# mgp25/OpenLTE

Measured on AMD Instinct MI355X. Metric: DL subframes/sec @20MHz 100RB 64QAM, full chain FFT->CE->demap->rate-unmatch->turbo(REF)->CRC (SURVEY 8d W4), higher is better.
Workload: dtype i8 IQ in, f32 FFT/CE/equaliser, i8 soft bits, i16 path metrics (differences exact modulo 2^16); 1 GPU; W4 full DL chain: 20 MHz/100 RB/64QAM, 9 allocations per subframe (8x12 PRB TBS 3240 + 1x4 PRB TBS 1064), 65536 subframes per GPU, int8 IQ in HBM; subframes_per_gpu=65536, N_ant=1, CFI=2, channel_estimate_form=compact, decoder=REF (reference-faithful, bit-exact), unique_subframes=96, streams_per_gpu=1

## Files before the change

openlte_amd/csrc/turbo.hip:

```cpp
#include <algorithm>
#include <cstring>
#include <type_traits>
#include <vector>

#include "plan_core.hpp"

namespace {

constexpr uint32_t RX_NULL_AS_INT = 10000;

__host__ __device__ inline uint32_t kpad64(uint32_t K) { return (K + 63u) & ~63u; }


__device__ __forceinline__ int sbyte(uint32_t w, int k) { return (int)__builtin_amdgcn_sbfe(w, 8 * k, 8); }

typedef __attribute__((address_space(3))) const uint8_t  lds_u8_t;
typedef __attribute__((address_space(3))) const int8_t   lds_i8_t;
typedef __attribute__((address_space(3))) const uint16_t lds_u16_t;
__device__ __forceinline__ uint32_t lds_u8(uint32_t addr) { return *(lds_u8_t *)(uintptr_t)addr; }
__device__ __forceinline__ int      lds_i8(uint32_t addr) { return *(lds_i8_t *)(uintptr_t)addr; }
__device__ __forceinline__ uint32_t lds_u16(uint32_t addr) { return *(lds_u16_t *)(uintptr_t)addr; }

typedef short v2s __attribute__((ext_vector_type(2)));
__device__ __forceinline__ v2s      as_v2s(uint32_t w) { return __builtin_bit_cast(v2s, w); }
__device__ __forceinline__ uint32_t as_u32(v2s v) { return __builtin_bit_cast(uint32_t, v); }
__device__ __forceinline__ v2s      even2(uint32_t w) { return (as_v2s(w) << 8) >> 8; }
__device__ __forceinline__ v2s      odd2(uint32_t w) { return as_v2s(w) >> 8; }
__device__ __forceinline__ uint32_t merge_bytes(v2s e, v2s o) { return __builtin_amdgcn_perm(as_u32(o), as_u32(e), 0x06020400u); }
__device__ __forceinline__ v2s      abs2(v2s a) { return __builtin_elementwise_max(a, (v2s)(0) - a); }
__device__ __forceinline__ uint32_t neg_mask(v2s d)
{
    uint32_t m;
    asm("v_pk_ashrrev_i16 %0, 15, %1 op_sel_hi:[0,1]" : "=v"(m) : "v"(as_u32(d)));
    return m;
}
__device__ __forceinline__ v2s bit_select(uint32_t m, v2s yes, v2s no) { return as_v2s((as_u32(yes) & m) | (as_u32(no) & ~m)); }
__device__ __forceinline__ v2s half_sum(v2s a, v2s b)
{
    uint32_t t = as_u32(a + b);
    asm("" : "+v"(t));
    return as_v2s(t) >> 1;
}

__device__ __forceinline__ int soft_xor(int a, int b)
{
    int mag = (abs(a) + abs(b)) >> 1;
    return ((a < 0) != (b < 0)) ? -mag : mag;
}


template <typename Op> __device__ __forceinline__ int wave_reduce_i(int v, Op op)
{
    v = op(v, __builtin_amdgcn_update_dpp(v, v, 0xB1, 0xF, 0xF, false));
    v = op(v, __builtin_amdgcn_update_dpp(v, v, 0x4E, 0xF, 0xF, false));
    v = op(v, __builtin_amdgcn_update_dpp(v, v, 0x141, 0xF, 0xF, false));
    v = op(v, __builtin_amdgcn_update_dpp(v, v, 0x140, 0xF, 0xF, false));
// ... 188 lines not shown
            nulls = __popc(mask0) + __popc(mask0 & lowmask(c + 1)) + __popc(mask2 & lowmask(cc));
        }
        cn = p - nulls;
    }
};

struct CbDesc { uint32_t alloc, e_off, E, combo, Nnn, hard, tbs, pad; };

struct GroupDesc {
    const mi_lte_pdsch_alloc *allocs;
    const uint32_t *cb_alloc;
    const int8_t   *e_base;
    const uint32_t *e_off;
    const uint32_t *e_len;
    uint8_t        *out_bits;
    uint32_t        out_stride;
    int32_t        *status;
    const uint32_t *crc_tab;
    uint32_t        ul;
    uint32_t        packed;
    const CbDesc   *desc;
};

struct KSeg {
    uint32_t        K, n_cb, cb_base, n_tiles;
    uint32_t        wg_cb;
    uint32_t        wg_perm, perm_grid;
    uint32_t        e_cap;
    uint32_t        wv1, wv23;
    uint64_t        arr_off;
    __attribute__((address_space(1))) const uint16_t *pi, *inv2, *tabs;
    __attribute__((address_space(1))) const uint32_t *nnn;
    uint32_t        ws1, ws23;
    uint64_t        pad;
};
static_assert(sizeof(KSeg) == 96, "KSeg is read with scalar loads: keep it a multiple of 16 bytes");
struct MultiArgs { const KSeg *segs; const uint32_t *map; };
typedef __attribute__((address_space(4))) const KSeg     const_seg_t;
typedef __attribute__((address_space(4))) const uint32_t const_map_t;
__device__ __forceinline__ const_seg_t &multi_seg(const MultiArgs &ma, uint32_t slot)
{
    const uint32_t idx = reinterpret_cast<const_map_t *>(reinterpret_cast<uintptr_t>(ma.map))[__builtin_amdgcn_readfirstlane(slot)];
    return reinterpret_cast<const_seg_t *>(reinterpret_cast<uintptr_t>(ma.segs))[idx];
}


struct SrcRateUnmatch {
    static constexpr bool kIntegerValued = true;
    uint32_t e_cap;
    GroupDesc       g;
    const uint16_t *tabs;
    const uint32_t *nnn;
    const uint16_t *tab;
    const int8_t   *e;
    uint32_t        E, Nnn, K_;
    __device__ __forceinline__ void seg(const_seg_fwd_t &sg);
    __device__ __forceinline__ void init(uint32_t cb, uint32_t K)
    {
        const_u32x4_t *dp = reinterpret_cast<const_u32x4_t *>(reinterpret_cast<uintptr_t>(g.desc + cb));
        const u32x4_t  d0 = dp[0], d1 = dp[1];
        tab = tabs + (size_t)d0.w * 3 * K;
        Nnn = d1.x;
        K_  = K;
        e   = g.e_base + (size_t)d0.y * 64;
        E   = d0.z;
        hard = d1.y != 0;
    }
// ... 912 lines not shown
        }
        __syncthreads();
        uint4 I1 = make_uint4(0, 0, 0, 0);
        if (nv > 0) {
            uint32_t idx[16];
            unpack_idx16(praw, idx);
            I1 = gather16_bytes(MTAB_N, idx);
        }
        if (nv >= 0) *reinterpret_cast<uint4 *>(a.out[0] + unit_off(tile_off, lane, u)) = I1;
        uint32_t w[16], wm = 0;
        if (nv <= 0) X2 = make_uint4(0, 0, 0, 0);
        abs_sum16(X2, I1, w, wm);
        const int   wmax = block_max_i((int)wm, red_i);
        if (wmax == 254 || wmax == 127) {
            uint32_t o[4];
#pragma unroll
            for (int j = 0; j < 4; j++) {
                const uint32_t p = pack4u(w[4 * j], w[4 * j + 1], w[4 * j + 2], w[4 * j + 3]);
                o[j] = wmax == 254 ? (p >> 1) & 0x7F7F7F7Fu : p;
            }
            if (nv >= 0) *reinterpret_cast<uint4 *>(a.out[1] + unit_off(tile_off, lane, u)) = make_uint4(o[0], o[1], o[2], o[3]);
            continue;
        }
        const float W = (float)wmax;
        for (uint32_t t = threadIdx.x; t < MTAB_N; t += blockDim.x) mtab[t] = (int8_t)(int)(127.0f * ((float)t / W));
        __syncthreads();
        if (nv >= 0) *reinterpret_cast<uint4 *>(a.out[1] + unit_off(tile_off, lane, u)) = lookup16(0, w);
        __syncthreads();
    }
}

struct VoteArgs { const uint8_t *X0, *A1, *B1, *B2; };

template <bool GROUP, int NSLOT, bool MULTI = false>
__global__ __launch_bounds__(384) __attribute__((amdgpu_waves_per_eu(6, 8))) void k_turbo_vote(VoteArgs a, uint32_t K_arg, uint32_t n_cb_arg, const uint16_t *__restrict__ inv_arg,
                                                    uint8_t *__restrict__ c_bits, GroupDesc g, MultiArgs ma)
{
    static_assert(NSLOT == 1, "one unit per thread");
    uint32_t K = K_arg, n_cb = n_cb_arg, bidx = blockIdx.x;
    size_t   seg_off = 0;
    const uint16_t *__restrict__ inv = inv_arg;
    if constexpr (MULTI) {
        const_seg_t &sg = multi_seg(ma, blockIdx.x >> 9);
        K = sg.K; n_cb = sg.n_cb; inv = (const uint16_t *)sg.inv2; bidx = blockIdx.x - sg.wg_cb; seg_off = sg.arr_off;
        g.desc += sg.cb_base;
    }
    extern __shared__ __attribute__((aligned(16))) int8_t sm[];
    const uint32_t cb = xcd_cb(bidx, n_cb), tile = cb >> 6, lane = cb & 63, Kp = kpad64(K), n_units = Kp >> 4;
    if (cb >= n_cb) return;
    const size_t   tile_off = seg_off + (size_t)tile * Kp * 64;
    int8_t        *d12 = sm, *bits = sm + 2 * Kp + 32;
    uint32_t      *red_u = reinterpret_cast<uint32_t *>(bits + Kp);
    const uint32_t u  = threadIdx.x;
    const int      nv = (u < n_units) ? min(16, max(0, (int)K - 16 * (int)u)) : -1;
    IdxRaw vraw;
    {
        const uint4 *ip = reinterpret_cast<const uint4 *>(inv + 16 * (size_t)(nv > 0 ? u : 0));
        vraw.lo = ip[0];
        vraw.hi = ip[1];
    }
    const uint32_t crc_w0 = (GROUP && nv > 0) ? g.crc_tab[MI_CRC_TAB_BIAS + K - 16 * u - 16] : 0u;
    v2s            s0e[4], s0o[4];
    if (threadIdx.x == 0) *reinterpret_cast<uint32_t *>(d12 + 2 * Kp) = 0u;
    if (nv >= 0) {
        const UnitWords wa = load_unit_words(a.A1, tile_off, lane, u), wb = load_unit_words(a.B1, tile_off, lane, u),
                        wc = load_unit_words(a.B2, tile_off, lane, u);
        WordPairs       pa = word_pairs(wa.w[0]), pb = word_pairs(wb.w[0]), pc = word_pairs(wc.w[0]);
        const uint4    x0 = *reinterpret_cast<const uint4 *>(a.X0 + unit_off(tile_off, lane, u));
        const uint32_t x0w[4] = {x0.x, x0.y, x0.z, x0.w};
        uint32_t       dn[8];
#pragma unroll
        for (int j = 0; j < 4; j++) {
            const WordPairs ca = word_pairs(wa.w[j + 1]), cb1 = word_pairs(wb.w[j + 1]), cb2 = word_pairs(wc.w[j + 1]);
            SX              fe, fo, ge, go, he, ho;
            feedback_sm(ca, pa, fe, fo);
            feedback_sm(cb1, pb, ge, go);
            feedback_sm(cb2, pc, he, ho);
            v2s d[2];
#pragma unroll
            for (int h = 0; h < 2; h++) {
                const SM  &A = h ? ca.o : ca.e, &B = h ? cb1.o : cb1.e, &B_ = h ? cb2.o : cb2.e;
                const SX  &G = h ? go : ge, &G_ = h ? ho : he;
                const v2s  At = h ? ca.ot : ca.et;
                const v2s dAG = At - G.tc, t = as_v2s(as_u32(dAG) ^ B.s) - as_v2s(B.s);
                const v2s v1  = bit_select(B.s ^ G.s, (v2s)(0) - (t >> 1), half_sum(B.m, G.m));
                const v2s v2  = bit_select(B_.s ^ G_.s, (v2s)(0) - ((B_.m - G_.tc) >> 1), half_sum(B_.m, G_.m));
                d[h] = v1 + v2;
                const v2s c1 = sxor_tc(A, h ? fo : fe);
                (h ? s0o[j] : s0e[j]) = (h ? odd2(x0w[j]) : even2(x0w[j])) + c1;
            }
            pa = ca; pb = cb1; pc = cb2;
            const bool in = 4 * j < nv;
            dn[2 * j]     = in ? __builtin_amdgcn_perm(as_u32(d[1]), as_u32(d[0]), 0x05040100u) : 0u;
            dn[2 * j + 1] = in ? __builtin_amdgcn_perm(as_u32(d[1]), as_u32(d[0]), 0x07060302u) : 0u;
        }
        uint4 *dst = reinterpret_cast<uint4 *>(d12 + 32 * u);
        dst[0] = make_uint4(dn[0], dn[1], dn[2], dn[3]);
        dst[1] = make_uint4(dn[4], dn[5], dn[6], dn[7]);
    } else {
#pragma unroll
        for (int j = 0; j < 4; j++) s0e[j] = s0o[j] = (v2s)(0);
    }
    __syncthreads();
    uint32_t alloc = 0, tbs = 0, F = 0, crc = 0;
    if (GROUP) {
        alloc = g.desc[cb].alloc;
        tbs   = g.desc[cb].tbs;
        F     = K - tbs - 24;
    }
    if (nv > 0) {
        const uint32_t  iw[8] = {vraw.lo.x, vraw.lo.y, vraw.lo.z, vraw.lo.w, vraw.hi.x, vraw.hi.y, vraw.hi.z, vraw.hi.w};
        uint32_t        me[4], mo[4], bw[4];
#pragma unroll
        for (int j = 0; j < 4; j++) {
            const uint32_t i0 = iw[2 * j] & 0xFFFFu, i1 = iw[2 * j] >> 16, i2 = iw[2 * j + 1] & 0xFFFFu, i3 = iw[2 * j + 1] >> 16;
            const uint32_t ge = lds_u16(i0) | lds_u16(i2) << 16, go = lds_u16(i1) | lds_u16(i3) << 16;
            me[j] = as_u32((s0e[j] + as_v2s(ge)) >> 15);
            mo[j] = as_u32((s0o[j] + as_v2s(go)) >> 15);
            bw[j] = (me[j] & 0x00010001u) | (mo[j] & 0x00010001u) << 8;
        }
        if (GROUP) {
            if (!(nv == 16 && 16 * u >= F)) {
#pragma unroll
                for (int j = 0; j < 4; j++) {
                    auto ok = [&](int k) { return (k < nv && 16 * u + k >= F) ? 0xFFFFu : 0u; };
                    me[j] &= ok(4 * j) | ok(4 * j + 2) << 16;
                    mo[j] &= ok(4 * j + 1) | ok(4 * j + 3) << 16;
                }
            }
            const uint32_t GS = 0x864CFBu << 8;
            uint32_t       w = crc_w0;
#pragma unroll
            for (int k = 15; k >= 0; k--) {
                const int      j = k >> 2;
                const uint32_t m = (k & 3) == 0 ? (uint32_t)__builtin_amdgcn_sbfe(me[j], 0, 1) : (k & 3) == 1 ? (uint32_t)__builtin_amdgcn_sbfe(mo[j], 0, 1)
                                 : (k & 3) == 2 ? (uint32_t)((int)me[j] >> 31) : (uint32_t)((int)mo[j] >> 31);
                crc ^= w & m;
                if (k > 0) w = (w << 1) ^ ((uint32_t)((int)w >> 31) & GS);
            }
        }
        const uint4 pk = make_uint4(bw[0], bw[1], bw[2], bw[3]);
        if (GROUP) *reinterpret_cast<uint4 *>(bits + 16 * u) = pk;
        else {
            uint2 *o = reinterpret_cast<uint2 *>(c_bits + (size_t)cb * K + 16 * u);
            o[0] = make_uint2(pk.x, pk.y);
            if (nv > 8) o[1] = make_uint2(pk.z, pk.w);
        }
    }
    if (GROUP) {
        crc = wave_xor_u(crc);
        __syncthreads();
        if ((threadIdx.x & 63) == 0) red_u[threadIdx.x >> 6] = crc;
        __syncthreads();
        crc = 0;
        for (uint32_t w = 0; w < (blockDim.x >> 6); w++) crc ^= red_u[w];
        if (threadIdx.x == 0) g.status[alloc] = (crc == 0) ? 0  : 2 ;
        uint8_t *o = g.out_bits + (size_t)alloc * g.out_stride;
        if (g.packed && ((F | tbs) & 7u) == 0) {
            const uint32_t nby = tbs >> 3, nw = nby >> 2;
            auto byte_at = [&](uint32_t m) -> uint32_t {
                const uint2 w = *reinterpret_cast<const uint2 *>(bits + F + 8 * m);
                return (((w.x * 0x08040201u) >> 24) & 0xFu) << 4 | (((w.y * 0x08040201u) >> 24) & 0xFu);
            };
            for (uint32_t m = threadIdx.x; m < nw; m += blockDim.x)
                reinterpret_cast<uint32_t *>(o)[m] = byte_at(4 * m) | byte_at(4 * m + 1) << 8 | byte_at(4 * m + 2) << 16 | byte_at(4 * m + 3) << 24;
            for (uint32_t m = 4 * nw + threadIdx.x; m < nby; m += blockDim.x) o[m] = (uint8_t)byte_at(m);
        } else if (g.packed) {
            for (uint32_t m = threadIdx.x; m < (tbs + 7) >> 3; m += blockDim.x) {
                uint32_t v = 0;
                for (uint32_t b = 0; b < 8; b++) v = v << 1 | ((8 * m + b < tbs) ? ((uint32_t)bits[F + 8 * m + b] & 1u) : 0u);
                o[m] = (uint8_t)v;
            }
        } else if ((F & 3u) == 0) {
            const uint32_t nq = tbs >> 2;
            const uint32_t *bw = reinterpret_cast<const uint32_t *>(bits + F);
            for (uint32_t m = threadIdx.x; m < nq; m += blockDim.x) reinterpret_cast<uint32_t *>(o)[m] = bw[m];
            for (uint32_t m = 4 * nq + threadIdx.x; m < tbs; m += blockDim.x) o[m] = (uint8_t)bits[m + F];
        } else
            for (uint32_t m = threadIdx.x; m < tbs; m += blockDim.x) o[m] = (uint8_t)bits[m + F];
    }
}

__global__ __launch_bounds__(256) void k_cb_desc(GroupDesc g, uint32_t n_cb, const uint32_t *__restrict__ nnn, CbDesc *__restrict__ out)
{
    const uint32_t cb = blockIdx.x * blockDim.x + threadIdx.x;
    if (cb >= n_cb) return;
    const uint32_t a = g.cb_alloc[cb], txm = g.allocs[a].tx_mode;
    const uint32_t combo = g.ul ? 8u + (g.allocs[a].rv_idx & 3u)
                                : ((g.allocs[a].rv_idx & 3u) << 1) | ((txm == 3 || txm == 4 || txm == 8 || txm == 9) ? 1u : 0u);
    CbDesc d;
    d.alloc = a; d.e_off = g.e_off[a]; d.E = g.e_len[a]; d.combo = combo; d.Nnn = nnn[combo];
    d.hard  = (g.allocs[a].mod_type >= 2 && d.E <= d.Nnn) ? 1u : 0u;
    d.tbs   = g.allocs[a].tbs; d.pad = 0;
    out[cb] = d;
}

__global__ __launch_bounds__(256) void k_cb_desc_multi(GroupDesc g, uint32_t n_cb, const KSeg *__restrict__ segs, uint32_t n_seg, CbDesc *__restrict__ out)
{
    const uint32_t cb = blockIdx.x * blockDim.x + threadIdx.x;
    if (cb >= n_cb) return;
    uint32_t lo = 0, hi = n_seg;
    while (hi - lo > 1) {
        const uint32_t mid = (lo + hi) >> 1;
        if (segs[mid].cb_base <= cb) lo = mid; else hi = mid;
    }
    const uint32_t a = g.cb_alloc[cb], txm = g.allocs[a].tx_mode;
    const uint32_t combo = g.ul ? 8u + (g.allocs[a].rv_idx & 3u)
                                : ((g.allocs[a].rv_idx & 3u) << 1) | ((txm == 3 || txm == 4 || txm == 8 || txm == 9) ? 1u : 0u);
    CbDesc d;
    d.alloc = a; d.e_off = g.e_off[a]; d.E = g.e_len[a]; d.combo = combo; d.Nnn = segs[lo].nnn[combo];
    d.hard  = (g.allocs[a].mod_type >= 2 && d.E <= d.Nnn) ? 1u : 0u;
    d.tbs   = g.allocs[a].tbs; d.pad = 0;
// ... 229 lines not shown

static bool no_static_lds(const void *kernel)
{
    hipFuncAttributes a;
    return hipFuncGetAttributes(&a, kernel) == hipSuccess && a.sharedSizeBytes == 0;
}

struct RefScratch {
    uint8_t *base;
    CbDesc  *d_desc;
    PrepOut  po;
    SisoArgs s1, s23;
    PermArgs pa;
    VoteArgs va;
    RefScratch(void *scratch, size_t arr_bytes) : base((uint8_t *)scratch)
    {
        uint8_t *arr[N_BYTE_ARRAYS];
        for (int a = 0; a < N_BYTE_ARRAYS; a++) arr[a] = base + a * arr_bytes;
        uint32_t *dec[3];
        for (int p = 0; p < 3; p++) dec[p] = (uint32_t *)(base + N_BYTE_ARRAYS * arr_bytes + p * (arr_bytes / 2));
        d_desc = (CbDesc *)(base + N_BYTE_ARRAYS * arr_bytes + 3 * (arr_bytes / 2));
        po.arr[0] = arr[AX0]; po.arr[1] = arr[AX1]; po.arr[2] = arr[AX2];
        po.arr[3] = arr[AI0]; po.arr[4] = arr[AM1]; po.arr[5] = arr[AM2];
        s1.p[0] = {arr[AX1], arr[AX0], arr[AM1], arr[AA1], dec[0]};
        s1.p[1] = s1.p[0];
        pa.A1 = arr[AA1]; pa.X2 = arr[AX2]; pa.out[0] = arr[AI1]; pa.out[1] = arr[AM3];
        s23.p[0] = {arr[AX2], arr[AI0], arr[AM2], arr[AB1], dec[1]};
        s23.p[1] = {arr[AX2], arr[AI1], arr[AM3], arr[AB2], dec[2]};
        va = {arr[AX0], arr[AA1], arr[AB1], arr[AB2]};
    }
};
static uint32_t gpw_of(uint32_t n_tr) { return n_tr <= 2048 ? 1u : n_tr <= 4096 ? 2u : n_tr <= 8192 ? 4u : SMALL_G; }

template <typename Src, bool GROUP>
static int turbo_ref_run(mi_lte_ctx *ctx, Src src, uint32_t K, uint32_t n_cb, uint8_t *d_c_bits, GroupDesc gd, uint32_t e_cap = 0)
{
    TurboTables tb;
    int         rc = mi_ctx_turbo_tables(ctx, K, 0, &tb);
    if (rc != MI_LTE_OK) return rc;
    static const bool lds_ok = no_static_lds((const void *)k_turbo_prep<Src, 1>) && no_static_lds((const void *)k_turbo_perm<1>) &&
                               no_static_lds((const void *)k_turbo_vote<GROUP, 1>);
    if (!lds_ok) {
        ctx->err = "turbo kernels were built with static LDS: absolute LDS addressing is invalid";
        return MI_LTE_ERR_HIP;
    }
    const size_t n_tiles = (n_cb + 63) / 64, Kp = kpad64(K), arr_bytes = n_tiles * Kp * 64;
    rc = mi_ctx_reserve_scratch(ctx, mi_lte_turbo_scratch_bytes(K, n_cb));
    if (rc != MI_LTE_OK) return rc;
    const RefScratch sc(ctx->scratch, arr_bytes);
    const bool small = n_cb <= ctx->siso_small_max;
    if (n_cb % 64 && !small)
        MI_HIP_CHECK(ctx, hipMemsetAsync(sc.base, 0, N_BYTE_ARRAYS * arr_bytes, ctx->stream));

    if constexpr (GROUP) {
        gd.desc = src.g.desc = sc.d_desc;
        MI_LAUNCH(ctx, "k_cb_desc", k_cb_desc, dim3((n_cb + 255) / 256), dim3(256), 0, gd, n_cb, (const uint32_t *)src.nnn, sc.d_desc);
    }
    const uint32_t cb_threads = (uint32_t)(((Kp >> 4) + 63) & ~(size_t)63);
    MI_LAUNCH(ctx, "k_turbo_prep", (k_turbo_prep<Src, 1>), dim3(8 * xcd_chunk(n_cb)), dim3(cb_threads), prep_lds_bytes(Kp, e_cap), src, K, n_cb, tb.d_pi, sc.po, MultiArgs{});

    auto lds_of = [&](uint32_t gpw) { return sizeof(uint32_t) * gpw * (64 * 4 * 2 + (Kp >> 5) * 4); };
    if (small)
        MI_LAUNCH(ctx, "k_turbo_siso_small", k_turbo_siso_small<false>, dim3((n_cb + gpw_of(n_cb) - 1) / gpw_of(n_cb)), dim3(64), lds_of(gpw_of(n_cb)), sc.s1, K, n_cb, 0u,
                  gpw_of(n_cb), MultiArgs{});
    else
        MI_LAUNCH(ctx, "k_turbo_siso", k_turbo_siso<false>, dim3(((n_tiles + 1) / 2 + 3) / 4), dim3(256), 0, sc.s1, K, (uint32_t)n_tiles, 0u, MultiArgs{}, (const uint32_t *)nullptr);

    const uint32_t perm_grid = ((8 * xcd_chunk(n_cb) + PERM_NB - 1) / PERM_NB + 7u) & ~7u;
    MI_LAUNCH(ctx, "k_turbo_perm", k_turbo_perm<1>, dim3(perm_grid), dim3(cb_threads), MTAB_N + Kp + 32, sc.pa, K, n_cb, tb.d_pi, MultiArgs{});

    if (small)
        MI_LAUNCH(ctx, "k_turbo_siso_small", k_turbo_siso_small<false>, dim3((2 * n_cb + gpw_of(2 * n_cb) - 1) / gpw_of(2 * n_cb)), dim3(64), lds_of(gpw_of(2 * n_cb)), sc.s23, K,
                  n_cb, 1u, gpw_of(2 * n_cb), MultiArgs{});
    else
        MI_LAUNCH(ctx, "k_turbo_siso", k_turbo_siso<false>, dim3((n_tiles + 3) / 4), dim3(256), 0, sc.s23, K, (uint32_t)n_tiles, 1u, MultiArgs{}, (const uint32_t *)nullptr);

    MI_LAUNCH(ctx, "k_turbo_vote", (k_turbo_vote<GROUP, 1>), dim3(8 * xcd_chunk(n_cb)), dim3(cb_threads), 3 * Kp + 64, sc.va, K, n_cb, tb.d_inv2, d_c_bits, gd, MultiArgs{});
    MI_HIP_CHECK(ctx, hipGetLastError());
    ctx->last_kernels = "k_turbo_prep:1,k_turbo_siso:2,k_turbo_perm:1,k_turbo_vote:1";
    return MI_LTE_OK;
}

template <typename T>
static int turbo_ref_batch(mi_lte_ctx *ctx, const T *d_soft, uint32_t K, uint32_t n_cb, uint8_t *d_c_bits)
{
    SrcDirect<T> src{0, d_soft, nullptr};
    GroupDesc    none{};
    return turbo_ref_run<SrcDirect<T>, false>(ctx, src, K, n_cb, d_c_bits, none);
}

static int rm_rank_tables(mi_lte_ctx *ctx, uint32_t K, RmTables *out)
{
    auto it = ctx->rm_tables.find(K);
    if (it == ctx->rm_tables.end()) {
        RmTables t;
        MI_HIP_CHECK(ctx, hipMalloc((void **)&t.d_tabs, sizeof(uint16_t) * 12 * 3 * K));
        MI_HIP_CHECK(ctx, hipMalloc((void **)&t.d_nnn, sizeof(uint32_t) * 12));
        ctx->owned.push_back(t.d_tabs);
        ctx->owned.push_back(t.d_nnn);
        MI_LAUNCH(ctx, "k_rm_rank_table", k_rm_rank_table, dim3((3 * K + 255) / 256, 12), dim3(256), 0, K, t.d_tabs, t.d_nnn);
        MI_HIP_CHECK(ctx, hipGetLastError());
        it = ctx->rm_tables.emplace(K, t).first;
    }
    *out = it->second;
    return MI_LTE_OK;
}

static GroupDesc group_desc(const mi_lte_ctx *ctx, const MiDecodeIO &io, uint32_t cb_base = 0)
{
    return {io.d_allocs, io.d_cb_alloc + cb_base, io.d_e, io.d_e_off, io.d_e_len, io.d_out_bits, io.out_stride, io.d_status, ctx->d_crc_tab, io.ul ? 1u : 0u, io.packed ? 1u : 0u};
}
static uint32_t stage_cap(uint32_t e_max_bytes) { return (e_max_bytes + 16u + 63u) & ~63u; }

static bool mi_turbo_ref_multi_takes(uint32_t K, uint32_t e_max_bytes) { return (e_max_bytes + (3 * K - 81) - 1) / (3 * K - 81) <= 258; }

static int mi_turbo_ref_group(mi_lte_ctx *ctx, const MiKGroup &gr, const MiDecodeIO &io)
{
    int rc = mi_ctx_crc_table(ctx);
    if (rc != MI_LTE_OK) return rc;
    const GroupDesc gd = group_desc(ctx, io, gr.cb_base);
    RmTables rt;
    rc = rm_rank_tables(ctx, gr.K, &rt);
    if (rc != MI_LTE_OK) return rc;
    SrcRateUnmatch src;
    src.g    = gd;
    src.tabs = rt.d_tabs;
    src.nnn  = rt.d_nnn;
    const uint32_t cap = stage_cap(gr.e_max);
    src.e_cap          = (prep_lds_bytes(kpad64(gr.K), cap) <= 48 * 1024) ? cap : 0;
    if (mi_turbo_ref_multi_takes(gr.K, gr.e_max)) {
        SrcRateUnmatchPk pk;
        static_cast<SrcRateUnmatch &>(pk) = src;
        return turbo_ref_run<SrcRateUnmatchPk, true>(ctx, pk, gr.K, gr.n_cb, nullptr, gd, src.e_cap);
    }
    return turbo_ref_run<SrcRateUnmatch, true>(ctx, src, gr.K, gr.n_cb, nullptr, gd, src.e_cap);
}

static int mi_turbo_ref_multi(mi_lte_ctx *ctx, const MiKGroup *groups, uint32_t n_groups, const MiDecodeIO &io, MiMultiCache *cache)
{
    if (!groups || n_groups == 0 || n_groups > 0xFFFF || !cache) return MI_LTE_ERR_INVALID_ARG;
    int rc = mi_ctx_crc_table(ctx);
    if (rc != MI_LTE_OK) return rc;
    static const bool lds_ok = no_static_lds((const void *)k_turbo_prep<SrcRateUnmatchPk, 1, true>) && no_static_lds((const void *)k_turbo_perm<1, true>) &&
                               no_static_lds((const void *)k_turbo_vote<true, 1, true>);
    if (!lds_ok) { ctx->err = "turbo kernels were built with static LDS: absolute LDS addressing is invalid"; return MI_LTE_ERR_HIP; }
    constexpr int NCLS = 6;
    auto cls_of = [](uint32_t K) { return (int)((((kpad64(K) >> 4) + 63) >> 6) - 1); };
    const bool same = cache->built_for.size() == n_groups && memcmp(cache->built_for.data(), groups, sizeof(MiKGroup) * n_groups) == 0;
    if (!same) {
        cache->built_for.clear();
        std::vector<KSeg>     segs(n_groups);
        std::vector<uint32_t> map;
        MiMultiGeom          &G = cache->geom;
        G = MiMultiGeom{};
        uint64_t arr = 0;
        uint32_t cbs = 0;
        for (uint32_t i = 0; i < n_groups; i++) {
            const MiKGroup &gr = groups[i];
            if ((i && gr.K <= groups[i - 1].K) || gr.n_cb == 0) { ctx->err = "merged decode: groups must be non-empty and in ascending block size"; return MI_LTE_ERR_INVALID_ARG; }
            TurboTables tb;
            RmTables    rt;
            if ((rc = mi_ctx_turbo_tables(ctx, gr.K, 0, &tb)) != MI_LTE_OK || (rc = rm_rank_tables(ctx, gr.K, &rt)) != MI_LTE_OK) return rc;
            KSeg &sg = segs[i];
            memset(&sg, 0, sizeof(sg));
            const uint32_t Kp = kpad64(gr.K), cap = stage_cap(gr.e_max);
            sg.K = gr.K; sg.n_cb = gr.n_cb; sg.cb_base = gr.cb_base; sg.n_tiles = (gr.n_cb + 63) / 64;
            const uint32_t cap_w = (uint32_t)((15 * (size_t)(gr.K + 4) / 4 + 64 + 63) & ~(size_t)63);
            sg.e_cap = (prep_lds_bytes(Kp, cap) <= 48 * 1024) ? (Kp <= 1024 ? std::min(cap, cap_w) : cap) : cap_w;
            sg.arr_off = arr;
            typedef __attribute__((address_space(1))) const uint16_t gl16_t;
            typedef __attribute__((address_space(1))) const uint32_t gl32_t;
            sg.pi = (gl16_t *)tb.d_pi; sg.inv2 = (gl16_t *)tb.d_inv2; sg.tabs = (gl16_t *)rt.d_tabs; sg.nnn = (gl32_t *)rt.d_nnn;
            arr += (uint64_t)sg.n_tiles * Kp * 64;
            cbs = std::max(cbs, gr.cb_base + gr.n_cb);
            const int c = cls_of(gr.K);
            G.one_size[c] = (G.lds_prep[c] == 0 && gr.n_cb % 64 == 0) ? (int)i : -1;
            G.off_one[c] = sg.arr_off; G.e_cap_one[c] = sg.e_cap;
// ... 48 lines not shown
            const uint32_t n_wg = (n_wv + 3) / 4;
            if (!many_sizes || n_wg < 512) return;
            *at = (uint32_t)map.size();
            for (uint32_t j = 0; j < n_wg; j++) {
                const uint32_t round = j / 256, c = j % 256, in_round = std::min(256u, n_wg - 256 * round);
                const uint32_t src = (round & 1u) ? 256 * round + (in_round - 1 - std::min(c, in_round - 1)) : j;
                for (uint32_t t = 0; t < 4; t++) map.push_back(4 * src + t < n_wv ? 4 * src + t : 0xFFFFFFFFu);
            }
            *n_out = 4 * n_wg;
        };
        deal(G.n_wv1, &G.ord_wv1, &G.n_ord1);
        deal(G.n_wv23, &G.ord_wv23, &G.n_ord23);
        uint32_t tot = 0, kp_all = 0;
        for (uint32_t i = 0; i < n_groups; i++) { tot += groups[i].n_cb; kp_all = std::max(kp_all, kpad64(groups[i].K)); }
        G.gpw1 = gpw_of(tot); G.gpw23 = gpw_of(2 * tot); G.kp_all = kp_all;
        G.map_ws1 = (uint32_t)map.size();
        uint32_t wg = 0;
        for (uint32_t i = 0; i < n_groups; i++) {
            const uint32_t n = (groups[i].n_cb + G.gpw1 - 1) / G.gpw1;
            segs[i].ws1 = wg;
            map.insert(map.end(), n, i);
            wg += n;
        }
        G.n_ws1   = wg;
        G.map_ws23 = (uint32_t)map.size();
        wg = 0;
        for (uint32_t i = 0; i < n_groups; i++) {
            const uint32_t n = (2 * groups[i].n_cb + G.gpw23 - 1) / G.gpw23;
            segs[i].ws23 = wg;
            map.insert(map.end(), n, i);
            wg += n;
        }
        G.n_ws23 = wg;
        const size_t seg_bytes = sizeof(KSeg) * n_groups, map_bytes = (sizeof(uint32_t) * map.size() + 15) & ~(size_t)15, need = seg_bytes + map_bytes;
        if (need > cache->cap) {
            MI_HIP_CHECK(ctx, hipStreamSynchronize(ctx->stream));
            if (cache->d_tab) (void)hipFree(cache->d_tab);
            cache->d_tab = nullptr; cache->cap = 0;
            MI_HIP_CHECK(ctx, hipMalloc(&cache->d_tab, need + need / 4));
            cache->cap = need + need / 4;
        }
        std::vector<uint8_t> blob(need, 0);
        memcpy(blob.data(), segs.data(), seg_bytes);
        memcpy(blob.data() + seg_bytes, map.data(), sizeof(uint32_t) * map.size());
        MI_H2D(ctx, cache->d_tab, blob.data(), need);
        G.map_off = seg_bytes;
        cache->built_for.assign(groups, groups + n_groups);
    }
    const MiMultiGeom &G = cache->geom;
    const size_t A = G.arr_bytes;
    rc = mi_ctx_reserve_scratch(ctx, N_BYTE_ARRAYS * A + 3 * (A / 2) + (size_t)((G.n_slots + 63) & ~63u) * sizeof(CbDesc));
    if (rc != MI_LTE_OK) return rc;
    const RefScratch sc(ctx->scratch, A);
    const KSeg     *d_segs = (const KSeg *)cache->d_tab;
    const uint32_t *d_map  = (const uint32_t *)((const uint8_t *)cache->d_tab + G.map_off);

    GroupDesc gd = group_desc(ctx, io);
    gd.desc = sc.d_desc;
    MI_LAUNCH(ctx, "k_cb_desc", k_cb_desc_multi, dim3((G.n_slots + 255) / 256), dim3(256), 0, gd, G.n_slots, d_segs, n_groups, sc.d_desc);
    SrcRateUnmatchPk src;
    src.g = gd; src.tabs = nullptr; src.nnn = nullptr; src.e_cap = 0;
    for (int c = 0; c < NCLS; c++)
        if (G.grid_cb[c]) {
            if (G.one_size[c] >= 0) {
                const MiKGroup &gr = groups[G.one_size[c]];
                TurboTables tb;
                RmTables    rt;
                if ((rc = mi_ctx_turbo_tables(ctx, gr.K, 0, &tb)) != MI_LTE_OK || (rc = rm_rank_tables(ctx, gr.K, &rt)) != MI_LTE_OK) return rc;
                SrcRateUnmatchPk s1 = src;
                s1.tabs = rt.d_tabs; s1.nnn = rt.d_nnn; s1.g.desc = sc.d_desc + gr.cb_base; s1.e_cap = G.e_cap_one[c];
                PrepOut p1 = sc.po;
                for (int a = 0; a < 6; a++) p1.arr[a] += G.off_one[c];
                MI_LAUNCH(ctx, "k_turbo_prep", (k_turbo_prep<SrcRateUnmatchPk, 1, false>), dim3(G.grid_cb[c]), dim3(64 * (c + 1)), G.lds_prep[c], s1, gr.K, gr.n_cb, (const uint16_t *)tb.d_pi,
                          p1, MultiArgs{});
                continue;
            }
            MI_LAUNCH(ctx, "k_turbo_prep", (k_turbo_prep<SrcRateUnmatchPk, 1, true>), dim3(G.grid_cb[c]), dim3(64 * (c + 1)), G.lds_prep[c], src, 0u, 0u, (const uint16_t *)nullptr, sc.po,
                      (MultiArgs{d_segs, d_map + G.map_cb[c]}));
        }
    const bool small = G.n_slots <= ctx->siso_small_max;
    auto lds_small = [&](uint32_t gpw) { return sizeof(uint32_t) * gpw * (64 * 4 * 2 + (G.kp_all >> 5) * 4); };
    if (small)
        MI_LAUNCH(ctx, "k_turbo_siso_small", k_turbo_siso_small<true>, dim3(G.n_ws1), dim3(64), lds_small(G.gpw1), sc.s1, 0u, 0u, 0u, G.gpw1, (MultiArgs{d_segs, d_map + G.map_ws1}));
    else
    MI_LAUNCH(ctx, "k_turbo_siso", k_turbo_siso<true>, dim3(G.n_ord1 ? G.n_ord1 / 4 : (G.n_wv1 + 3) / 4), dim3(256), G.siso_pad1, sc.s1, 0u, G.n_wv1, 0u, (MultiArgs{d_segs, d_map + G.map_wv1}),
              G.n_ord1 ? d_map + G.ord_wv1 : (const uint32_t *)nullptr);
    for (int c = 0; c < NCLS; c++)
        if (G.grid_perm[c])
            MI_LAUNCH(ctx, "k_turbo_perm", (k_turbo_perm<1, true>), dim3(G.grid_perm[c]), dim3(64 * (c + 1)), MTAB_N + G.kp_max[c] + 32, sc.pa, 0u, 0u, (const uint16_t *)nullptr,
                      (MultiArgs{d_segs, d_map + G.map_perm[c]}));
    if (small)
        MI_LAUNCH(ctx, "k_turbo_siso_small", k_turbo_siso_small<true>, dim3(G.n_ws23), dim3(64), lds_small(G.gpw23), sc.s23, 0u, 0u, 1u, G.gpw23, (MultiArgs{d_segs, d_map + G.map_ws23}));
    else
    MI_LAUNCH(ctx, "k_turbo_siso", k_turbo_siso<true>, dim3(G.n_ord23 ? G.n_ord23 / 4 : (G.n_wv23 + 3) / 4), dim3(256), G.siso_pad23, sc.s23, 0u, G.n_wv23, 1u, (MultiArgs{d_segs, d_map + G.map_wv23}),
              G.n_ord23 ? d_map + G.ord_wv23 : (const uint32_t *)nullptr);
    for (int c = 0; c < NCLS; c++)
        if (G.grid_cb[c])
            MI_LAUNCH(ctx, "k_turbo_vote", (k_turbo_vote<true, 1, true>), dim3(G.grid_cb[c]), dim3(64 * (c + 1)), 3 * G.kp_max[c] + 64, sc.va, 0u, 0u, (const uint16_t *)nullptr,
                      (uint8_t *)nullptr, gd, (MultiArgs{d_segs, d_map + G.map_cb[c]}));
    MI_HIP_CHECK(ctx, hipGetLastError());
    return MI_LTE_OK;
}

int mi_turbo_ref_dispatch(mi_lte_ctx *ctx, const MiKGroup *groups, uint32_t n_groups, const MiDecodeIO &io, MiMultiCache *cache)
{
    std::vector<MiKGroup> take;
    if (ctx->merged_decode)
        for (uint32_t i = 0; i < n_groups; i++)
            if (mi_turbo_ref_multi_takes(groups[i].K, groups[i].e_max)) take.push_back(groups[i]);
    const bool merged = take.size() >= 2;
    int        rc;
    if (merged && (rc = mi_turbo_ref_multi(ctx, take.data(), (uint32_t)take.size(), io, cache)) != MI_LTE_OK) return rc;
    for (uint32_t i = 0; i < n_groups; i++) {
        const MiKGroup &gr = groups[i];
        if (merged && mi_turbo_ref_multi_takes(gr.K, gr.e_max)) continue;
        rc = mi_turbo_ref_group(ctx, gr, io);
        if (rc != MI_LTE_OK) return rc;
    }
    ctx->last_kernels = !merged                 ? "k_turbo_prep,k_turbo_siso,k_turbo_perm,k_turbo_vote per block size"
                        : take.size() == n_groups ? "k_cb_desc:1,k_turbo_prep,k_turbo_siso:2,k_turbo_perm,k_turbo_vote per workgroup width over all block sizes"
                                                  : "k_cb_desc:1,k_turbo_prep,k_turbo_siso:2,k_turbo_perm,k_turbo_vote per workgroup width over all block sizes but the per-size ones";
    return MI_LTE_OK;
}

void mi_multi_cache_free(MiMultiCache *cache)
{
    if (cache && cache->d_tab) (void)hipFree(cache->d_tab);
    if (cache) { cache->d_tab = nullptr; cache->cap = 0; cache->built_for.clear(); }
}

int mi_turbo_bcjr_group(mi_lte_ctx *ctx, const MiKGroup &gr, const MiDecodeIO &io, int8_t *d_soft, uint8_t *d_c_bits, uint32_t mode, uint32_t n_iter, int qpp_spec)
{
    const uint32_t K = gr.K, n_cb = gr.n_cb;
    int rc = mi_ctx_crc_table(ctx);
    if (rc != MI_LTE_OK) return rc;
    GroupDesc gd = group_desc(ctx, io, gr.cb_base);
    RmTables  t;
    rc = rm_rank_tables(ctx, K, &t);
    if (rc != MI_LTE_OK) return rc;
    const uint32_t cap = stage_cap(gr.e_max), e_cap = cap <= 60 * 1024 ? cap : 0;
    if (mode == MI_LTE_TURBO_BCJR_BLOCK) {
        MI_LAUNCH(ctx, "k_rm_to_i8", k_rm_to_i8, dim3(n_cb), dim3(256), e_cap, gd, K, n_cb, (const uint16_t *)t.d_tabs, (const uint32_t *)t.d_nnn, d_soft, e_cap);
        MI_HIP_CHECK(ctx, hipGetLastError());
        rc = mi_turbo_bcjr_block_batch(ctx, d_soft, K, n_cb, n_iter, qpp_spec, d_c_bits);
    } else {
        static const bool lds_ok = no_static_lds((const void *)k_rm_bcjr_prep);
        if (!lds_ok) { ctx->err = "k_rm_bcjr_prep was built with static LDS"; return MI_LTE_ERR_HIP; }
        TurboTables tb;
        rc = mi_ctx_turbo_tables(ctx, K, qpp_spec ? 1 : 0, &tb);
        if (rc != MI_LTE_OK) return rc;
        MiBcjrBufs mb;
        rc = mi_turbo_bcjr_begin(ctx, K, n_cb, &mb);
        if (rc != MI_LTE_OK) return rc;
        const size_t   Kp = kpad64(K);
// ... 54 lines not shown
```

Measured before the change: 2.711 million subframes/s.

## Pack several small code blocks per workgroup in turbo vote kernel

Lets k_turbo_vote process 2 or 4 code blocks per workgroup when K is small, so lanes that were idle padding in partially filled waves do useful work. Each packed block gets its own LDS region, with offset-adjusted interleaver indices and a per-slot CRC reduction. The merged-decode path gains new vote classes with their own map entries and segment offsets. The price is extra index arithmetic and more complex reduction and dispatch logic.

```diff
diff --git a/openlte_amd/csrc/turbo.hip b/openlte_amd/csrc/turbo.hip
--- a/openlte_amd/csrc/turbo.hip
+++ b/openlte_amd/csrc/turbo.hip
@@ -22,6 +22,7 @@
 __device__ __forceinline__ uint32_t lds_u16(uint32_t addr) { return *(lds_u16_t *)(uintptr_t)addr; }
 
 typedef short v2s __attribute__((ext_vector_type(2)));
+typedef unsigned short v2us __attribute__((ext_vector_type(2)));
 __device__ __forceinline__ v2s      as_v2s(uint32_t w) { return __builtin_bit_cast(v2s, w); }
 __device__ __forceinline__ uint32_t as_u32(v2s v) { return __builtin_bit_cast(uint32_t, v); }
 __device__ __forceinline__ v2s      even2(uint32_t w) { return (as_v2s(w) << 8) >> 8; }
@@ -276,7 +277,8 @@
     __attribute__((address_space(1))) const uint16_t *pi, *inv2, *tabs;
     __attribute__((address_space(1))) const uint32_t *nnn;
     uint32_t        ws1, ws23;
-    uint64_t        pad;
+    uint32_t        wg_vote;
+    uint32_t        pad;
 };
 static_assert(sizeof(KSeg) == 96, "KSeg is read with scalar loads: keep it a multiple of 16 bytes");
 struct MultiArgs { const KSeg *segs; const uint32_t *map; };
@@ -1255,27 +1257,37 @@
 
 struct VoteArgs { const uint8_t *X0, *A1, *B1, *B2; };
 
-template <bool GROUP, int NSLOT, bool MULTI = false>
-__global__ __launch_bounds__(384) __attribute__((amdgpu_waves_per_eu(6, 8))) void k_turbo_vote(VoteArgs a, uint32_t K_arg, uint32_t n_cb_arg, const uint16_t *__restrict__ inv_arg,
+template <bool GROUP, int NSLOT, bool MULTI = false, int NB = 1>
+__global__ __launch_bounds__(NB == 1 ? 384 : 256) __attribute__((amdgpu_waves_per_eu(6, 8))) void k_turbo_vote(VoteArgs a, uint32_t K_arg, uint32_t n_cb_arg, const uint16_t *__restrict__ inv_arg,
                                                     uint8_t *__restrict__ c_bits, GroupDesc g, MultiArgs ma)
 {
     static_assert(NSLOT == 1, "one unit per thread");
+    static_assert(NB == 1 || NB == 2 || NB == 4, "a size's grid is a multiple of the merged decode's map granularity (512 / NB workgroups) for the divisors of 64");
     uint32_t K = K_arg, n_cb = n_cb_arg, bidx = blockIdx.x;
     size_t   seg_off = 0;
     const uint16_t *__restrict__ inv = inv_arg;
     if constexpr (MULTI) {
-        const_seg_t &sg = multi_seg(ma, blockIdx.x >> 9);
-        K = sg.K; n_cb = sg.n_cb; inv = (const uint16_t *)sg.inv2; bidx = blockIdx.x - sg.wg_cb; seg_off = sg.arr_off;
+        const_seg_t &sg = multi_seg(ma, blockIdx.x >> (NB == 1 ? 9 : NB == 2 ? 8 : 7));
+        K = sg.K; n_cb = sg.n_cb; inv = (const uint16_t *)sg.inv2; bidx = blockIdx.x - sg.wg_vote; seg_off = sg.arr_off;
         g.desc += sg.cb_base;
     }
     extern __shared__ __attribute__((aligned(16))) int8_t sm[];
-    const uint32_t cb = xcd_cb(bidx, n_cb), tile = cb >> 6, lane = cb & 63, Kp = kpad64(K), n_units = Kp >> 4;
-    if (cb >= n_cb) return;
+    const uint32_t Kp = kpad64(K), n_units = Kp >> 4;
+    const uint32_t cb0 = NB == 1 ? xcd_cb(bidx, n_cb) : (bidx & 7u) * xcd_chunk(n_cb) + (bidx >> 3) * NB;
+    if (cb0 >= n_cb) return;
+    uint32_t       b = 0, u = threadIdx.x;
+    if constexpr (NB > 1) {
+#pragma unroll
+        for (int i = 1; i <= NB; i++) b += (threadIdx.x >= i * n_units) ? 1u : 0u;
+        u = threadIdx.x - b * n_units;
+    }
+    const uint32_t cb = cb0 + b, tile = cb0 >> 6, lane = (cb0 & 63) + b;
+    const bool     live = NB == 1 || (b < NB && cb < n_cb);
+    const uint32_t region = 3 * Kp + 64, lbase = NB == 1 ? 0u : b * region;
     const size_t   tile_off = seg_off + (size_t)tile * Kp * 64;
-    int8_t        *d12 = sm, *bits = sm + 2 * Kp + 32;
+    int8_t        *d12 = sm + lbase, *bits = d12 + 2 * Kp + 32;
     uint32_t      *red_u = reinterpret_cast<uint32_t *>(bits + Kp);
-    const uint32_t u  = threadIdx.x;
-    const int      nv = (u < n_units) ? min(16, max(0, (int)K - 16 * (int)u)) : -1;
+    const int      nv = (live && u < n_units) ? min(16, max(0, (int)K - 16 * (int)u)) : -1;
     IdxRaw vraw;
     {
         const uint4 *ip = reinterpret_cast<const uint4 *>(inv + 16 * (size_t)(nv > 0 ? u : 0));
@@ -1284,7 +1296,7 @@
     }
     const uint32_t crc_w0 = (GROUP && nv > 0) ? g.crc_tab[MI_CRC_TAB_BIAS + K - 16 * u - 16] : 0u;
     v2s            s0e[4], s0o[4];
-    if (threadIdx.x == 0) *reinterpret_cast<uint32_t *>(d12 + 2 * Kp) = 0u;
+    if (NB == 1 ? threadIdx.x == 0 : (live && u == 0)) *reinterpret_cast<uint32_t *>(d12 + 2 * Kp) = 0u;
     if (nv >= 0) {
         const UnitWords wa = load_unit_words(a.A1, tile_off, lane, u), wb = load_unit_words(a.B1, tile_off, lane, u),
                         wc = load_unit_words(a.B2, tile_off, lane, u);
@@ -1324,15 +1336,27 @@
 #pragma unroll
         for (int j = 0; j < 4; j++) s0e[j] = s0o[j] = (v2s)(0);
     }
+    uint32_t alloc = 0, tbs = 0, F = 0, crc = 0;
+    if constexpr (GROUP && NB > 1) {
+        if (live) {
+            alloc = g.desc[cb].alloc;
+            tbs   = g.desc[cb].tbs;
+            F     = K - tbs - 24;
+        }
+    }
     __syncthreads();
-    uint32_t alloc = 0, tbs = 0, F = 0, crc = 0;
-    if (GROUP) {
+    if constexpr (GROUP && NB == 1) {
         alloc = g.desc[cb].alloc;
         tbs   = g.desc[cb].tbs;
         F     = K - tbs - 24;
     }
     if (nv > 0) {
-        const uint32_t  iw[8] = {vraw.lo.x, vraw.lo.y, vraw.lo.z, vraw.lo.w, vraw.hi.x, vraw.hi.y, vraw.hi.z, vraw.hi.w};
+        uint32_t        iw[8] = {vraw.lo.x, vraw.lo.y, vraw.lo.z, vraw.lo.w, vraw.hi.x, vraw.hi.y, vraw.hi.z, vraw.hi.w};
+        if constexpr (NB > 1) {
+            const v2us base2 = (v2us)((unsigned short)lbase);
+#pragma unroll
+            for (int k = 0; k < 8; k++) iw[k] = __builtin_bit_cast(uint32_t, __builtin_bit_cast(v2us, iw[k]) + base2);
+        }
         uint32_t        me[4], mo[4], bw[4];
 #pragma unroll
         for (int j = 0; j < 4; j++) {
@@ -1371,13 +1395,35 @@
         }
     }
     if (GROUP) {
-        crc = wave_xor_u(crc);
-        __syncthreads();
-        if ((threadIdx.x & 63) == 0) red_u[threadIdx.x >> 6] = crc;
-        __syncthreads();
-        crc = 0;
-        for (uint32_t w = 0; w < (blockDim.x >> 6); w++) crc ^= red_u[w];
-        if (threadIdx.x == 0) g.status[alloc] = (crc == 0) ? 0  : 2 ;
+        if constexpr (NB == 1) {
+            crc = wave_xor_u(crc);
+            __syncthreads();
+            if ((threadIdx.x & 63) == 0) red_u[threadIdx.x >> 6] = crc;
+            __syncthreads();
+            crc = 0;
+            for (uint32_t w = 0; w < (blockDim.x >> 6); w++) crc ^= red_u[w];
+        } else {
+            auto slot_of = [&](uint32_t t) {
+                uint32_t s = 0;
+#pragma unroll
+                for (int i = 1; i <= NB; i++) s += (t >= i * n_units) ? 1u : 0u;
+                return s;
+            };
+            const uint32_t wave = __builtin_amdgcn_readfirstlane(threadIdx.x >> 6);
+            const uint32_t s_lo = slot_of(64 * wave), s_hi = min(slot_of(64 * wave + 63), (uint32_t)NB - 1);
+            for (uint32_t s = s_lo; s <= s_hi; s++) {
+                const uint32_t x = wave_xor_u(b == s ? crc : 0u);
+                if ((threadIdx.x & 63) == 0) reinterpret_cast<uint32_t *>(sm + s * region + 3 * Kp + 32)[wave - ((s * n_units) >> 6)] = x;
+            }
+            __syncthreads();
+            crc = 0;
+            if (live) {
+                const uint32_t nw = (((b + 1) * n_units - 1) >> 6) - ((b * n_units) >> 6) + 1;
+                for (uint32_t w = 0; w < nw; w++) crc ^= red_u[w];
+            }
+        }
+        const uint32_t stride = NB == 1 ? blockDim.x : n_units;
+        if (NB == 1 ? threadIdx.x == 0 : (live && u == 0)) g.status[alloc] = (crc == 0) ? 0  : 2 ;
         uint8_t *o = g.out_bits + (size_t)alloc * g.out_stride;
         if (g.packed && ((F | tbs) & 7u) == 0) {
             const uint32_t nby = tbs >> 3, nw = nby >> 2;
@@ -1385,11 +1431,11 @@
                 const uint2 w = *reinterpret_cast<const uint2 *>(bits + F + 8 * m);
                 return (((w.x * 0x08040201u) >> 24) & 0xFu) << 4 | (((w.y * 0x08040201u) >> 24) & 0xFu);
             };
-            for (uint32_t m = threadIdx.x; m < nw; m += blockDim.x)
+            for (uint32_t m = u; m < nw; m += stride)
                 reinterpret_cast<uint32_t *>(o)[m] = byte_at(4 * m) | byte_at(4 * m + 1) << 8 | byte_at(4 * m + 2) << 16 | byte_at(4 * m + 3) << 24;
-            for (uint32_t m = 4 * nw + threadIdx.x; m < nby; m += blockDim.x) o[m] = (uint8_t)byte_at(m);
+            for (uint32_t m = 4 * nw + u; m < nby; m += stride) o[m] = (uint8_t)byte_at(m);
         } else if (g.packed) {
-            for (uint32_t m = threadIdx.x; m < (tbs + 7) >> 3; m += blockDim.x) {
+            for (uint32_t m = u; m < (tbs + 7) >> 3; m += stride) {
                 uint32_t v = 0;
                 for (uint32_t b = 0; b < 8; b++) v = v << 1 | ((8 * m + b < tbs) ? ((uint32_t)bits[F + 8 * m + b] & 1u) : 0u);
                 o[m] = (uint8_t)v;
@@ -1397,10 +1443,10 @@
         } else if ((F & 3u) == 0) {
             const uint32_t nq = tbs >> 2;
             const uint32_t *bw = reinterpret_cast<const uint32_t *>(bits + F);
-            for (uint32_t m = threadIdx.x; m < nq; m += blockDim.x) reinterpret_cast<uint32_t *>(o)[m] = bw[m];
-            for (uint32_t m = 4 * nq + threadIdx.x; m < tbs; m += blockDim.x) o[m] = (uint8_t)bits[m + F];
+            for (uint32_t m = u; m < nq; m += stride) reinterpret_cast<uint32_t *>(o)[m] = bw[m];
+            for (uint32_t m = 4 * nq + u; m < tbs; m += stride) o[m] = (uint8_t)bits[m + F];
         } else
-            for (uint32_t m = threadIdx.x; m < tbs; m += blockDim.x) o[m] = (uint8_t)bits[m + F];
+            for (uint32_t m = u; m < tbs; m += stride) o[m] = (uint8_t)bits[m + F];
     }
 }
 
@@ -1696,6 +1742,68 @@
 };
 static uint32_t gpw_of(uint32_t n_tr) { return n_tr <= 2048 ? 1u : n_tr <= 4096 ? 2u : n_tr <= 8192 ? 4u : SMALL_G; }
 
+static uint32_t cb_threads_of(uint32_t K) { return ((kpad64(K) >> 4) + 63u) & ~63u; }
+
+constexpr uint32_t VOTE_NB_MAX = 4, VOTE_PACK_THREADS = 256;
+static uint32_t vote_lds_bytes(uint32_t Kp, uint32_t nb) { return nb * (3 * Kp + 64); }
+static uint32_t vote_nb(uint32_t K)
+{
+    const uint32_t n = kpad64(K) >> 4;
+    uint32_t best = 1, cost = 4 * ((n + 63) / 64);
+    for (uint32_t nb = 2; nb <= VOTE_NB_MAX; nb *= 2) {
+        const uint32_t waves = (nb * n + 63) / 64, c = 4 * waves / nb;
+        if (64 * waves <= VOTE_PACK_THREADS && c < cost) { best = nb; cost = c; }
+    }
+    return best;
+}
+static uint32_t vote_threads(uint32_t K) { return (vote_nb(K) * (kpad64(K) >> 4) + 63u) & ~63u; }
+struct VoteCls { uint32_t nb, threads, grid, map, kp_max; };
+constexpr uint32_t VOTE_CLS_MAX = 3 * (VOTE_PACK_THREADS / 64) + 6;
+static uint32_t vote_cls_key(uint32_t K) { return (vote_nb(K) == 4 ? 2u : vote_nb(K) == 2 ? 1u : 0u) * 16 + vote_threads(K) / 64 - 1; }
+static uint32_t vote_classes(const MiKGroup *groups, uint32_t n_groups, uint32_t map_start, VoteCls (&cls)[VOTE_CLS_MAX], KSeg *segs = nullptr, std::vector<uint32_t> *map = nullptr)
+{
+    uint32_t grid[48] = {0}, kp[48] = {0}, n = 0;
+    for (uint32_t i = 0; i < n_groups; i++) {
+        const uint32_t k = vote_cls_key(groups[i].K);
+        if (segs) segs[i].wg_vote = grid[k];
+        grid[k] += 8 * xcd_chunk(groups[i].n_cb) / vote_nb(groups[i].K);
+        kp[k] = std::max(kp[k], kpad64(groups[i].K));
+    }
+    for (uint32_t k = 0; k < 48; k++)
+        if (grid[k]) {
+            const uint32_t nb = 1u << (k / 16);
+            cls[n++] = VoteCls{nb, 64 * (k % 16 + 1), grid[k], map_start, kp[k]};
+            map_start += grid[k] / (512 / nb);
+            for (uint32_t i = 0; map && i < n_groups; i++)
+                if (vote_cls_key(groups[i].K) == k) map->insert(map->end(), 8 * xcd_chunk(groups[i].n_cb) / nb / (512 / nb), i);
+        }
+    return n;
+}
+static std::string packed_note(const MiKGroup *groups, uint32_t n_groups)
+{
+    std::string v;
+    for (uint32_t nb = 1; nb <= VOTE_NB_MAX; nb *= 2)
+        for (uint32_t i = 0; i < n_groups; i++)
+            if (vote_nb(groups[i].K) == nb) { v += (v.empty() ? "" : "+") + std::to_string(nb); break; }
+    return "; packed blocks per workgroup: k_turbo_prep 1, k_turbo_perm 1, k_turbo_vote " + v;
+}
+
+template <bool GROUP, bool MULTI>
+static bool vote_no_static_lds()
+{
+    return no_static_lds((const void *)k_turbo_vote<GROUP, 1, MULTI, 1>) && no_static_lds((const void *)k_turbo_vote<GROUP, 1, MULTI, 2>) &&
+           no_static_lds((const void *)k_turbo_vote<GROUP, 1, MULTI, 4>);
+}
+template <bool GROUP, bool MULTI>
+static void launch_vote(mi_lte_ctx *ctx, uint32_t nb, uint32_t grid, uint32_t threads, uint32_t Kp_max, const VoteArgs &va, uint32_t K, uint32_t n_cb, const uint16_t *inv,
+                        uint8_t *d_c_bits, const GroupDesc &gd, const MultiArgs &ma)
+{
+    const uint32_t lds = vote_lds_bytes(Kp_max, nb);
+    if (nb == 4)      MI_LAUNCH(ctx, "k_turbo_vote", (k_turbo_vote<GROUP, 1, MULTI, 4>), dim3(grid), dim3(threads), lds, va, K, n_cb, inv, d_c_bits, gd, ma);
+    else if (nb == 2) MI_LAUNCH(ctx, "k_turbo_vote", (k_turbo_vote<GROUP, 1, MULTI, 2>), dim3(grid), dim3(threads), lds, va, K, n_cb, inv, d_c_bits, gd, ma);
+    else              MI_LAUNCH(ctx, "k_turbo_vote", (k_turbo_vote<GROUP, 1, MULTI, 1>), dim3(grid), dim3(threads), lds, va, K, n_cb, inv, d_c_bits, gd, ma);
+}
+
 template <typename Src, bool GROUP>
 static int turbo_ref_run(mi_lte_ctx *ctx, Src src, uint32_t K, uint32_t n_cb, uint8_t *d_c_bits, GroupDesc gd, uint32_t e_cap = 0)
 {
@@ -1703,7 +1811,7 @@
     int         rc = mi_ctx_turbo_tables(ctx, K, 0, &tb);
     if (rc != MI_LTE_OK) return rc;
     static const bool lds_ok = no_static_lds((const void *)k_turbo_prep<Src, 1>) && no_static_lds((const void *)k_turbo_perm<1>) &&
-                               no_static_lds((const void *)k_turbo_vote<GROUP, 1>);
+                               vote_no_static_lds<GROUP, false>();
     if (!lds_ok) {
         ctx->err = "turbo kernels were built with static LDS: absolute LDS addressing is invalid";
         return MI_LTE_ERR_HIP;
@@ -1720,7 +1828,7 @@
         gd.desc = src.g.desc = sc.d_desc;
         MI_LAUNCH(ctx, "k_cb_desc", k_cb_desc, dim3((n_cb + 255) / 256), dim3(256), 0, gd, n_cb, (const uint32_t *)src.nnn, sc.d_desc);
     }
-    const uint32_t cb_threads = (uint32_t)(((Kp >> 4) + 63) & ~(size_t)63);
+    const uint32_t cb_threads = cb_threads_of(K);
     MI_LAUNCH(ctx, "k_turbo_prep", (k_turbo_prep<Src, 1>), dim3(8 * xcd_chunk(n_cb)), dim3(cb_threads), prep_lds_bytes(Kp, e_cap), src, K, n_cb, tb.d_pi, sc.po, MultiArgs{});
 
     auto lds_of = [&](uint32_t gpw) { return sizeof(uint32_t) * gpw * (64 * 4 * 2 + (Kp >> 5) * 4); };
@@ -1739,9 +1847,10 @@
     else
         MI_LAUNCH(ctx, "k_turbo_siso", k_turbo_siso<false>, dim3((n_tiles + 3) / 4), dim3(256), 0, sc.s23, K, (uint32_t)n_tiles, 1u, MultiArgs{}, (const uint32_t *)nullptr);
 
-    MI_LAUNCH(ctx, "k_turbo_vote", (k_turbo_vote<GROUP, 1>), dim3(8 * xcd_chunk(n_cb)), dim3(cb_threads), 3 * Kp + 64, sc.va, K, n_cb, tb.d_inv2, d_c_bits, gd, MultiArgs{});
+    launch_vote<GROUP, false>(ctx, vote_nb(K), 8 * xcd_chunk(n_cb) / vote_nb(K), vote_threads(K), (uint32_t)Kp, sc.va, K, n_cb, tb.d_inv2, d_c_bits, gd, MultiArgs{});
     MI_HIP_CHECK(ctx, hipGetLastError());
-    ctx->last_kernels = "k_turbo_prep:1,k_turbo_siso:2,k_turbo_perm:1,k_turbo_vote:1";
+    const MiKGroup one{K, n_cb, 0, 0};
+    ctx->last_kernels = "k_turbo_prep:1,k_turbo_siso:2,k_turbo_perm:1,k_turbo_vote:1" + packed_note(&one, 1);
     return MI_LTE_OK;
 }
 
@@ -1806,7 +1915,7 @@
     int rc = mi_ctx_crc_table(ctx);
     if (rc != MI_LTE_OK) return rc;
     static const bool lds_ok = no_static_lds((const void *)k_turbo_prep<SrcRateUnmatchPk, 1, true>) && no_static_lds((const void *)k_turbo_perm<1, true>) &&
-                               no_static_lds((const void *)k_turbo_vote<true, 1, true>);
+                               vote_no_static_lds<true, true>();
     if (!lds_ok) { ctx->err = "turbo kernels were built with static LDS: absolute LDS addressing is invalid"; return MI_LTE_ERR_HIP; }
     constexpr int NCLS = 6;
     auto cls_of = [](uint32_t K) { return (int)((((kpad64(K) >> 4) + 63) >> 6) - 1); };
@@ -1921,6 +2030,8 @@
             wg += n;
         }
         G.n_ws23 = wg;
+        VoteCls vcls[VOTE_CLS_MAX];
+        (void)vote_classes(groups, n_groups, (uint32_t)map.size(), vcls, segs.data(), &map);
         const size_t seg_bytes = sizeof(KSeg) * n_groups, map_bytes = (sizeof(uint32_t) * map.size() + 15) & ~(size_t)15, need = seg_bytes + map_bytes;
         if (need > cache->cap) {
             MI_HIP_CHECK(ctx, hipStreamSynchronize(ctx->stream));
@@ -1983,10 +2094,11 @@
     else
     MI_LAUNCH(ctx, "k_turbo_siso", k_turbo_siso<true>, dim3(G.n_ord23 ? G.n_ord23 / 4 : (G.n_wv23 + 3) / 4), dim3(256), G.siso_pad23, sc.s23, 0u, G.n_wv23, 1u, (MultiArgs{d_segs, d_map + G.map_wv23}),
               G.n_ord23 ? d_map + G.ord_wv23 : (const uint32_t *)nullptr);
-    for (int c = 0; c < NCLS; c++)
-        if (G.grid_cb[c])
-            MI_LAUNCH(ctx, "k_turbo_vote", (k_turbo_vote<true, 1, true>), dim3(G.grid_cb[c]), dim3(64 * (c + 1)), 3 * G.kp_max[c] + 64, sc.va, 0u, 0u, (const uint16_t *)nullptr,
-                      (uint8_t *)nullptr, gd, (MultiArgs{d_segs, d_map + G.map_cb[c]}));
+    VoteCls vcls[VOTE_CLS_MAX];
+    const uint32_t n_vcls = vote_classes(groups, n_groups, G.map_ws23 + G.n_ws23, vcls);
+    for (uint32_t v = 0; v < n_vcls; v++)
+        launch_vote<true, true>(ctx, vcls[v].nb, vcls[v].grid, vcls[v].threads, vcls[v].kp_max, sc.va, 0u, 0u, (const uint16_t *)nullptr, (uint8_t *)nullptr, gd,
+                                (MultiArgs{d_segs, d_map + vcls[v].map}));
     MI_HIP_CHECK(ctx, hipGetLastError());
     return MI_LTE_OK;
 }
@@ -2009,6 +2121,7 @@
     ctx->last_kernels = !merged                 ? "k_turbo_prep,k_turbo_siso,k_turbo_perm,k_turbo_vote per block size"
                         : take.size() == n_groups ? "k_cb_desc:1,k_turbo_prep,k_turbo_siso:2,k_turbo_perm,k_turbo_vote per workgroup width over all block sizes"
                                                   : "k_cb_desc:1,k_turbo_prep,k_turbo_siso:2,k_turbo_perm,k_turbo_vote per workgroup width over all block sizes but the per-size ones";
+    ctx->last_kernels += packed_note(groups, n_groups);
     return MI_LTE_OK;
 }
 
```

After: 2.710 million subframes/s. No clear change (-0.0%).
